# votnhan/VN_celeb_face_recognition

Hardware: AMD Instinct MI355X
Metric: embeddings/sec @ bs=256 (InceptionResnetV1, 160x160) (higher is better)
Workload: dtype bf16

## Files before the change

vn_celeb_face_recognition_amd/csrc/engine.h:

```cpp
#pragma once
#include <hip/hip_runtime.h>
#include <stdint.h>

#include <string>
#include <unordered_map>
#include <vector>

#include "../../include/vnface.h"
#include "kernels.h"

namespace vnf {

void set_error(const std::string& msg);
int fail(int code, const std::string& msg);
const char* last_error_cstr();

#define VNF_HIP(expr)                                                                         \
  do {                                                                                        \
    hipError_t _e = (expr);                                                                   \
    if (_e != hipSuccess)                                                                     \
      return ::vnf::fail(VNF_E_HIP, std::string(#expr) + ": " + hipGetErrorString(_e));       \
  } while (0)

enum class HandleKind { Encoder = 1, Mlp, Mtcnn, MlpTrainer, Retina, HeadTrainer, ConvProbe, Gallery };

struct HandleBase {
  const HandleKind kind;
  explicit HandleBase(HandleKind k) : kind(k) {}
  int device = 0;
  std::vector<void*> allocs;
  virtual ~HandleBase();
  void* dalloc(size_t bytes);
  void* upload(const void* host, size_t bytes);
};

template <class T>
T* handle_cast(vnf_handle h) {
  HandleBase* b = reinterpret_cast<HandleBase*>(h);
  return (b && b->kind == T::KIND) ? static_cast<T*>(b) : nullptr;
}

template <class T>
T* handle_cast_base(vnf_handle h) {
  HandleBase* b = reinterpret_cast<HandleBase*>(h);
  if (b)
    for (HandleKind k : T::KINDS)
      if (b->kind == k) return static_cast<T*>(b);
  return nullptr;
}

struct WeightMap {
  std::unordered_map<std::string, const vnf_tensor_desc*> m;
  std::string missing;
  WeightMap(const vnf_tensor_desc* w, int n);
  const float* get(const std::string& name, int64_t numel);
  bool has(const std::string& name) const { return m.count(name) != 0; }
};

void convert_to(int dtype, const float* src, void* dst, size_t n);

struct Buf {
  int H, W, C;
  size_t elems_per_image() const { return (size_t)H * W * C; }
  char* ptr = nullptr;
};

struct ConvLayer {
  std::string name;
  int x_buf, x_coff, cin;
  int H, W, Ho, Wo, KH, KW, sh, sw, ph, pw;
  void* w = nullptr;
  float* bias = nullptr;
  float* slope = nullptr;
  int4* ktab = nullptr;
  int K, Kpad, cout, cout_pad, ncls = 1;
  int nseg = 0;
  struct { int c0, c1, buf, coff; } seg[4];
  int res_buf = -1, res_coff = 0;
  int act = ACT_NONE, out_f32 = 0;
  int cfg = -1;
  double macs_alg = 0, macs_exec = 0;
};

struct Op {
  enum Kind { PACK, CONV, MAXPOOL, AVGPOOL, L2NORM, COPYOUT, STEM1, DWCONV, UPADD, RSTEM, DWPW, HEADS, SE } kind;
  int src = -1;
  int dst = -1, dst_coff = 0;
  int layer = -1;
  int res = -1;
  PoolWindow window = {0, 0, false};
  int frame_h = 0, frame_w = 0;
  int n_cls = 0, n_proj = 0, proj_col = 0;

  static Op pack(int dst) { Op o{PACK}; o.dst = dst; return o; }
  static Op conv(int layer) { Op o{CONV}; o.layer = layer; return o; }
  static Op stem1(int layer, int dst) { Op o{STEM1}; o.layer = layer; o.dst = dst; return o; }
  static Op maxpool(int src, int dst, int dst_coff, PoolWindow w = {3, 0, false}) {
    Op o{MAXPOOL}; o.src = src; o.dst = dst; o.dst_coff = dst_coff; o.window = w; return o;
  }
  static Op maxpool_ceil(int src, int dst, int k) { return maxpool(src, dst, 0, {k, 0, true}); }
  static Op maxpool_pad1(int src, int dst) { return maxpool(src, dst, 0, {3, 1, false}); }
  static Op avgpool(int src, int dst) { Op o{AVGPOOL}; o.src = src; o.dst = dst; return o; }
  static Op l2norm() { return Op{L2NORM}; }
  static Op copyout() { return Op{COPYOUT}; }
  static Op dwconv(int layer) { Op o{DWCONV}; o.layer = layer; return o; }
  static Op dwpw(int layer) { Op o{DWPW}; o.layer = layer; return o; }
  static Op upadd(int src, int dst) { Op o{UPADD}; o.src = src; o.dst = dst; return o; }
  static Op rstem(int frame_h, int frame_w, int dst) { Op o{RSTEM}; o.frame_h = frame_h; o.frame_w = frame_w; o.dst = dst; return o; }
  static Op se(int layer, int src, int res, int dst) { Op o{SE}; o.layer = layer; o.src = src; o.res = res; o.dst = dst; return o; }
  static Op heads(int n_cls, int n_proj, int proj_col) { Op o{HEADS}; o.n_cls = n_cls; o.n_proj = n_proj; o.proj_col = proj_col; return o; }
};

struct DwLayer {
  int x_buf, o_buf, C, stride;
  float *w = nullptr, *bias = nullptr;
  float slope = 0.f;
};

struct DwPwLayer {
  int x_buf, o_buf, cin, cout, stride;
  float *dw = nullptr, *dbias = nullptr, *pw = nullptr, *pbias = nullptr;
  float slope = 0.f;
  std::string name;
};

struct SeLayer {
  std::string name;
  int C, part_buf;
  float *w1 = nullptr, *b1 = nullptr, *w2 = nullptr, *b2 = nullptr;
  float slope_se = 0.f, slope_out = 0.f;
};

struct Group { int first, last, chunk; };

struct FusedStack {
  enum class Kind { StemMid, Block35, Block17 } kind = Kind::Block17;
  int first = 0, last = 0;
  int in_buf = -1, out_buf = -1;
  int nblocks = 0;
  int conv0 = 0;
  void* wstream = nullptr;
  float* bias = nullptr;
  void* wtail = nullptr;
  bool active = false;
  bool stack = false;
  double macs_alg = 0;
  int ext_last = 0, ext_conv = -1, ext_out_buf = -1;
  bool ext = false;
  int end() const { return ext ? ext_last : last; }
};

struct Tap { int buf, coff, C; };

struct EncoderEnv {
  int fuse = 31, direct_stem = 1, stem1a_mfma = 2, retina_fuse = 3, ws_persist = 1;
  int stem_chunk = 0, ir100_chunk1 = 0, ir100_chunk2 = 0;
  int autotune = 1, force_cfg = -2, tune_lanes = 0, autotune_log = 0;
  bool tune_final = true;
  std::string tune_cache;
  static EncoderEnv read();
};

struct RunExtra {
  float* out2 = nullptr;
  const uint8_t* prep_src = nullptr;
  int prep_s = 0;
};

constexpr int ARCH_MLP = -1, ARCH_RNET = -2, ARCH_ONET = -3, ARCH_RETINA = -5;

struct Encoder : HandleBase {
  static constexpr HandleKind KIND = HandleKind::Encoder;
  Encoder() : HandleBase(KIND) {}
  ~Encoder() override;
  int arch, dtype, max_batch, in_size;
  std::vector<Buf> bufs;
  std::vector<ConvLayer> convs;
  std::vector<DwLayer> dws;
  std::vector<DwPwLayer> dwpws;
  std::vector<SeLayer> ses;
  float *rstem_wa = nullptr, *rstem_bias = nullptr;
  std::vector<Op> ops;
  std::vector<Group> groups;
  std::vector<FusedStack> fused;
  std::vector<int> fused_at;
  int prepare_fused();
  int launch_fused(const FusedStack& f, int n0, int nn, hipStream_t s);
  std::unordered_map<std::string, Tap> taps;
  bool buf_materialised(int buf) const;
  float* emb_raw = nullptr;
  int emb_ld = 512;
  int n_cls = 0, n_proj = 0;
  float* cls_buf = nullptr;
  double macs_alg = 0, macs_exec = 0;
  Encoder* head = nullptr;
  int head_classes = 0, head_in = -1, head_logit = -1;
  float* head_emb = nullptr;
  hipEvent_t head_done = nullptr;

  int add_buf(int H, int W, int C);
  char* at(int buf, int n0, int coff = 0) const {
    return bufs[buf].ptr + ((size_t)n0 * bufs[buf].elems_per_image() + coff) * dtype_size(dtype);
  }
  float* at_f32(int buf, int n0) const { return (float*)at(buf, n0); }
  int finalize();
  int autotune();
  ConvArgs conv_args(const ConvLayer& L, int n0, int nn) const;
  int run(const void* x, int n, int x_dtype, float* out, hipStream_t s, std::string* report = nullptr,
          const RunExtra* extra = nullptr);
  int run_range(const void* x, int i0, int i1, int x_dtype, float* out, hipStream_t s, std::string* report, const RunExtra* extra);
  int write_report(std::vector<hipEvent_t>& prof_ev, const std::vector<int>& prof_op, int n, hipStream_t s, std::string* report) const;
  float* stem_wt = nullptr;
  int n_ctx = 1, next_ctx = 0;
  std::vector<std::vector<char*>> ctx_bufs;
  std::vector<float*> ctx_emb;
  std::vector<hipEvent_t> ctx_ev;
  int select_ctx(hipStream_t s, int* used);
  int max_streams = 4;
  bool tune_dirty = true;
  int tune_lanes = 1;
  int tune_batch = 0;
  const EncoderEnv env = EncoderEnv::read();
  hipStream_t side[4] = {nullptr, nullptr, nullptr, nullptr};
  hipEvent_t join_ev[4] = {nullptr, nullptr, nullptr, nullptr}, fork_ev = nullptr;
};

const char* fused_label(const FusedStack& f);
const char* fused_detail(const FusedStack& f);

int build_irv1(Encoder& e, WeightMap& wm);
int build_ir100(Encoder& e, WeightMap& wm);
int build_seir101(Encoder& e, WeightMap& wm);
int build_rn50_2b(Encoder& e, WeightMap& wm, int num_classes, int num_projections);
int build_retina_mnet(Encoder& e, WeightMap& wm, int H, int W, int head_bufs[3]);
struct NetBufs { int crops, pooled1, pooled2, heads; };
int build_rnet(Encoder& e, WeightMap& wm, bool mid, NetBufs& nb);
int build_onet(Encoder& e, WeightMap& wm, bool mid, NetBufs& nb);

}
```

vn_celeb_face_recognition_amd/csrc/fused.cpp:

```cpp
#include "engine.h"
#include "block35.h"
#include "stem_mid.h"
#include "trunk17.h"

#include <cstring>

namespace vnf {

using Kind = FusedStack::Kind;

int Encoder::prepare_fused() {
  const int enabled = env.fuse;
  for (FusedStack& f : fused) {
    f.active = false;
    if (!enabled || (dtype != BF16 && dtype != F16 && dtype != F16P) || f.nblocks < 1 || f.nblocks > T17_MAX_BLOCKS) continue;
    if (f.kind == Kind::StemMid) {
      if (!(enabled & 4)) continue;
      const ConvLayer& c2a = convs[f.conv0];
      const ConvLayer& c2b = convs[f.conv0 + 1];
      if (c2a.cout != 32 || c2a.K != 288 || c2b.cout != 64 || c2b.K != 288 || c2a.ncls != 1 || c2b.ncls != 1)
        return fail(VNF_E_INVALID, "fused stem: unexpected layer shapes");
      StemMidPack pk;
      pk.w[0] = c2a.w; pk.kpad[0] = c2a.Kpad;
      pk.w[1] = c2b.w; pk.kpad[1] = c2b.Kpad;
      bool ext_ok = false;
      if ((enabled & 8) && f.ext_conv >= 0) {
        const ConvLayer& c3b = convs[f.ext_conv];
        ext_ok = c3b.cout == 80 && c3b.K == 64 && c3b.KH == 1 && c3b.ncls == 1 && c3b.nseg == 1 && c3b.res_buf < 0 && c3b.act == ACT_RELU &&
                 bufs[f.ext_out_buf].C == 80;
      }
      if (dtype == F16P && !ext_ok) continue;
      f.wstream = dalloc(dtype == F16P ? SMS_WFRAG_BYTES : SM_WFRAG_BYTES);
      f.bias = (float*)dalloc(SM_BIAS * 4);
      if (!f.wstream || !f.bias) return VNF_E_HIP;
      VNF_HIP(hipMemcpy(f.bias, c2a.bias, 32 * 4, hipMemcpyDeviceToDevice));
      VNF_HIP(hipMemcpy(f.bias + 32, c2b.bias, 64 * 4, hipMemcpyDeviceToDevice));
      VNF_HIP(dtype == F16P ? stem_mids_repack(pk, f.wstream, 0) : stem_mid_repack(pk, f.wstream, 0));
      VNF_HIP(hipDeviceSynchronize());
      f.macs_alg = c2a.macs_alg + c2b.macs_alg;
      f.active = true;
      f.ext = ext_ok;
      if (ext_ok) f.macs_alg += convs[f.ext_conv].macs_alg;
      continue;
    }
    if (f.kind == Kind::Block35) {
      if (!(enabled & 2)) continue;
      std::vector<float> bias((size_t)f.nblocks * B35_BIAS, 0.f);
      static const int rows[5] = {96, 32, 32, 32, 256}, ks[5] = {256, 288, 288, 288, 96}, boff[5] = {0, 96, 128, 160, 192};
      const size_t wimg_bytes = dtype == F16P ? B35S_WIMG_BYTES : B35_WIMG_BYTES;
      f.wstream = dalloc((size_t)f.nblocks * wimg_bytes);
      f.bias = (float*)dalloc(bias.size() * 4);
      if (!f.wstream || !f.bias) return VNF_E_HIP;
      for (int b = 0; b < f.nblocks; ++b) {
        Block35Pack pk;
        pk.bias = f.bias + (size_t)b * B35_BIAS;
        for (int c = 0; c < 5; ++c) {
          const ConvLayer& L = convs[f.conv0 + 5 * b + c];
          if (L.cout != rows[c] || L.K != ks[c] || L.ncls != 1) return fail(VNF_E_INVALID, "fused Block35: unexpected layer shapes");
          pk.w[c] = L.w;
          pk.kpad[c] = L.Kpad;
          VNF_HIP(hipMemcpy(&bias[(size_t)b * B35_BIAS + boff[c]], L.bias, (size_t)rows[c] * 4, hipMemcpyDeviceToHost));
          f.macs_alg += L.macs_alg;
        }
        VNF_HIP(hipMemcpy(f.bias + (size_t)b * B35_BIAS, &bias[(size_t)b * B35_BIAS], (size_t)B35_BIAS * 4, hipMemcpyHostToDevice));
        VNF_HIP(dtype == F16P ? block35s_repack(pk, (char*)f.wstream + (size_t)b * wimg_bytes, 0)
                              : block35_repack(pk, (char*)f.wstream + (size_t)b * wimg_bytes, 0));
      }
      VNF_HIP(hipDeviceSynchronize());
      f.active = true;
      f.stack = (enabled & 16) && dtype != F16P;
      f.ext = false;
      if (f.stack && (enabled & 32) && f.ext_conv >= 0) {
        const ConvLayer& t = convs[f.ext_conv];
        const ConvLayer& last_up = convs[f.conv0 + 5 * (f.nblocks - 1) + 4];
        const bool ok = t.KH == 1 && t.KW == 1 && t.K == 256 && t.cout == 192 && t.ncls == 1 && t.nseg == 1 && t.res_buf < 0 &&
                        t.act == ACT_RELU && !t.out_f32 && t.x_buf == last_up.seg[0].buf && t.x_coff == 0 &&
                        t.seg[0].buf == f.ext_out_buf && t.seg[0].coff == 0 && bufs[f.ext_out_buf].C == 192;
        if (ok) {
          f.wtail = dalloc(B35_TAIL_BYTES);
          if (!f.wtail) return VNF_E_HIP;
          VNF_HIP(block35_tail_repack(t.w, t.Kpad, t.bias, f.wtail, 0));
          VNF_HIP(hipDeviceSynchronize());
          f.ext = true;
          f.macs_alg += t.macs_alg;
        }
      }
      continue;
    }
    if (!(enabled & 1)) continue;
    Trunk17Pack pk;
    memset(&pk, 0, sizeof pk);
    pk.nblocks = f.nblocks;
    std::vector<float> bias((size_t)f.nblocks * T17_BIAS, 0.f);
    static const int rows[4] = {256, 128, 128, 896}, ks[4] = {896, 896, 896, 256}, boff[4] = {0, 256, 384, 512};
    bool ok = true;
    for (int b = 0; b < f.nblocks && ok; ++b)
      for (int c = 0; c < 4 && ok; ++c) {
        const ConvLayer& L = convs[f.conv0 + 4 * b + c];
        if (L.cout != rows[c] || L.K != ks[c] || L.Kpad != ks[c] || L.ncls != 1) { ok = false; break; }
        pk.w[b][c] = L.w;
        pk.kpad[c] = L.Kpad;
        VNF_HIP(hipMemcpy(&bias[(size_t)b * T17_BIAS + boff[c]], L.bias, (size_t)rows[c] * 4, hipMemcpyDeviceToHost));
        f.macs_alg += L.macs_alg;
      }
    if (!ok) return fail(VNF_E_INVALID, "fused Block17 stack: unexpected layer shapes");
    f.wstream = dalloc(dtype == F16P ? trunk17s_stream_bytes(f.nblocks) : trunk17_stream_bytes(f.nblocks));
    f.bias = (float*)upload(bias.data(), bias.size() * 4);
    if (!f.wstream || !f.bias) return VNF_E_HIP;
    VNF_HIP(dtype == F16P ? trunk17s_repack(pk, f.wstream, 0) : trunk17_repack(pk, f.wstream, 0));
    VNF_HIP(hipDeviceSynchronize());
    f.active = true;
  }
  return VNF_OK;
}

bool Encoder::buf_materialised(int buf) const {
  for (const FusedStack& f : fused) {
    if (!f.active) continue;
    bool written = false;
    for (int oi = f.first; oi < f.end(); ++oi) {
      const Op& op = ops[oi];
      if (op.kind == Op::CONV) {
        const ConvLayer& L = convs[op.layer];
        for (int i = 0; i < L.nseg; ++i) written |= L.seg[i].buf == buf;
      } else if (op.kind == Op::MAXPOOL) {
        written |= op.dst == buf;
      }
    }
    if (!written) continue;
    bool produced = false;
    switch (f.kind) {
      case Kind::StemMid: produced = buf == (f.ext ? f.ext_out_buf : f.out_buf); break;
      case Kind::Block35:
        for (int b = 0; b < f.nblocks; ++b) produced |= convs[f.conv0 + 5 * b + 4].seg[0].buf == buf;
        produced |= f.ext && buf == f.ext_out_buf;
        break;
      case Kind::Block17: produced = buf == f.out_buf; break;
    }
    if (!produced) return false;
  }
  return true;
}

int Encoder::launch_fused(const FusedStack& f, int n0, int nn, hipStream_t s) {
  hipError_t err = hipSuccess;
  const char* what = "";
  switch (f.kind) {
    case Kind::StemMid: {
      const int out = f.ext ? f.ext_out_buf : f.out_buf;
      StemMidArgs sa;
      sa.x = at(f.in_buf, n0); sa.ldx = bufs[f.in_buf].C;
      sa.y = at(out, n0); sa.ldy = bufs[out].C;
      sa.n = nn;
      sa.wfrag = f.wstream; sa.bias = f.bias;
      sa.w3b = nullptr; sa.b3b = nullptr; sa.k3b_pad = 0;
      if (f.ext) {
        const ConvLayer& c3b = convs[f.ext_conv];
        sa.w3b = c3b.w; sa.b3b = c3b.bias; sa.k3b_pad = c3b.Kpad;
      }
      what = "fused stem";
      err = dtype == F16P ? launch_stem_mids(sa, s) : launch_stem_mid(sa, dtype, s);
      break;
    }
    case Kind::Block35:
      if (f.stack) {
        const int in = convs[f.conv0 + 4].res_buf;
        const int out = convs[f.conv0 + 5 * (f.nblocks - 1) + 4].seg[0].buf;
        Block35StackArgs ba;
        ba.x = at(in, n0); ba.ldx = bufs[in].C;
        ba.y = at(out, n0); ba.ldy = bufs[out].C;
        ba.n = nn; ba.nblocks = f.nblocks;
        ba.wimg = f.wstream;
        if (f.ext) {
          ba.wtail = f.wtail;
          ba.ytail = at(f.ext_out_buf, n0);
          ba.ldyt = bufs[f.ext_out_buf].C;
        }
        what = "fused Block35 stack";
        err = launch_block35_stack(ba, dtype, s);
        break;
      }
      what = "fused Block35";
      for (int b = 0; b < f.nblocks && err == hipSuccess; ++b) {
        const ConvLayer& up = convs[f.conv0 + 5 * b + 4];
        Block35Args ba;
        ba.x = at(up.res_buf, n0); ba.ldx = bufs[up.res_buf].C;
        ba.y = at(up.seg[0].buf, n0); ba.ldy = bufs[up.seg[0].buf].C;
        ba.n = nn;
        ba.wimg = (const char*)f.wstream + (size_t)b * (dtype == F16P ? B35S_WIMG_BYTES : B35_WIMG_BYTES);
        ba.zero = conv_zero_page();
        err = dtype == F16P ? launch_block35s(ba, s) : launch_block35(ba, dtype, s);
      }
      break;
    case Kind::Block17: {
      Trunk17Args ta;
      ta.x = at(f.in_buf, n0); ta.ldx = bufs[f.in_buf].C;
      ta.y = at(f.out_buf, n0); ta.ldy = bufs[f.out_buf].C;
      ta.n = nn; ta.nblocks = f.nblocks;
      ta.wstream = f.wstream; ta.bias = f.bias;
      what = "fused Block17 stack";
      err = dtype == F16P ? launch_trunk17s(ta, s) : launch_trunk17(ta, dtype, s);
      break;
    }
  }
  return err == hipSuccess ? VNF_OK : fail(VNF_E_HIP, std::string(what) + ": " + hipGetErrorString(err));
}

const char* fused_label(const FusedStack& f) {
  if (f.kind == Kind::StemMid) return f.ext ? "conv2d_2a+2b+maxpool_3a+3b" : "conv2d_2a+2b+maxpool_3a";
  return f.kind == Kind::Block35 ? "repeat_1 (fused blocks)" : "repeat_2 (persistent trunk)";
}

const char* fused_detail(const FusedStack& f) {
  if (f.kind == Kind::StemMid) return "rolling rows, one launch, one workgroup per image";
  if (f.kind == Kind::Block17) return "10 x Block17 in one launch, one workgroup per image";
  if (!f.stack) return "5 x Block35, one launch per block, one workgroup per image";
  return f.ext ? "5 x Block35 + mixed_6a.branch1.0 in one launch, x in registers"
               : "5 x Block35 in one launch, x in registers, one workgroup per image";
}

}
```

vn_celeb_face_recognition_amd/csrc/plan_irv1.cpp:

```cpp
#include "plan.h"

namespace vnf {

static bool basic_piece(WeightMap& wm, const std::string& p, int cin, int cout, int kh, int kw, Piece& out) {
  return fill_piece(wm, out, p + ".conv.weight", cout, cin * kh * kw, Epilogue::batchnorm(p + ".bn", 1e-3f));
}

int build_irv1(Encoder& e, WeightMap& wm) {
  e.in_size = 160;
  const int b_in = e.add_buf(160, 160, 8);
  const int b_1a = e.add_buf(79, 79, 32), b_2a = e.add_buf(77, 77, 32), b_2b = e.add_buf(77, 77, 64);
  const int b_3a = e.add_buf(38, 38, 64), b_3b = e.add_buf(38, 38, 80), b_4a = e.add_buf(36, 36, 192);
  const int x35[3] = {e.add_buf(17, 17, 256), e.add_buf(17, 17, 256), e.add_buf(17, 17, 256)};
  const int t35a = e.add_buf(17, 17, 64), t35b = e.add_buf(17, 17, 32), cat35 = e.add_buf(17, 17, 96);
  const int m6a = e.add_buf(17, 17, 192), m6b = e.add_buf(17, 17, 192);
  const int x17[3] = {e.add_buf(8, 8, 896), e.add_buf(8, 8, 896), e.add_buf(8, 8, 896)};
  const int t17a = e.add_buf(8, 8, 128), t17b = e.add_buf(8, 8, 128), cat17 = e.add_buf(8, 8, 256);
  const int m7a = e.add_buf(8, 8, 768), m7b = e.add_buf(8, 8, 256);
  const int x8[3] = {e.add_buf(3, 3, 1792), e.add_buf(3, 3, 1792), e.add_buf(3, 3, 1792)};
  const int t8a = e.add_buf(3, 3, 192), t8b = e.add_buf(3, 3, 192), cat8 = e.add_buf(3, 3, 384);
  const int pool = e.add_buf(1, 1, 1792);

  e.ops.push_back(Op::pack(b_in));

  auto simple = [&](const std::string& name, int xb, int xoff, int cin, int cin_pad, int cout, int kh, int kw, int st,
                    int ph, int pw, int ob, int ooff) -> int {
    ConvSpec s;
    s.name = name; s.x_buf = xb; s.x_coff = xoff; s.cin = cin; s.cin_pad = cin_pad;
    s.KH = kh; s.KW = kw; s.sh = s.sw = st; s.ph = ph; s.pw = pw;
    NEED(single_piece(wm, s, name + ".conv.weight", cout, ob, ooff, Epilogue::batchnorm(name + ".bn", 1e-3f)));
    return add_conv(e, s);
  };
  auto fused1x1 = [&](const std::string& name, std::vector<std::string> prefixes, int xb, int cin, int cout_each,
                      std::vector<SegSpec> segs) -> int {
    ConvSpec s;
    s.name = name; s.x_buf = xb; s.cin = s.cin_pad = cin;
    s.pieces.resize(prefixes.size());
    for (size_t i = 0; i < prefixes.size(); ++i)
      NEED(basic_piece(wm, prefixes[i], cin, cout_each, 1, 1, s.pieces[i]));
    s.segs = segs;
    return add_conv(e, s);
  };
  auto up = [&](const std::string& p, int cat, int cin, int cout, float scale, int xin, int xout, bool relu) -> int {
    ConvSpec s;
    s.name = p + ".conv2d"; s.x_buf = cat; s.cin = s.cin_pad = cin;
    NEED(single_piece(wm, s, p + ".conv2d.weight", cout, xout, 0, Epilogue::biased(p + ".conv2d.bias")));
    Piece& pc = s.pieces[0];
    pc.scale.assign(cout, scale);
    for (int i = 0; i < cout; ++i) pc.bias[i] = pc.bias[i] * scale;
    s.res_buf = xin;
    s.act = relu ? ACT_RELU : ACT_NONE;
    return add_conv(e, s);
  };

  TRY(simple("conv2d_1a", b_in, 0, 3, 8, 32, 3, 3, 2, 0, 0, b_1a, 0));
  {
    const int direct = e.env.direct_stem;
    Piece pc;
    if (direct && basic_piece(wm, "conv2d_1a", 3, 32, 3, 3, pc)) {
      std::vector<float> wt(27 * 32 + 32);
      for (int co = 0; co < 32; ++co) {
        for (int k = 0; k < 27; ++k) wt[k * 32 + co] = pc.w[co * 27 + k] * pc.scale[co];
        wt[27 * 32 + co] = pc.bias[co];
      }
      e.stem_wt = (float*)e.upload(wt.data(), wt.size() * 4);
      if (!e.stem_wt) return VNF_E_HIP;
      e.ops.resize(e.ops.size() - 2);
      e.ops.push_back(Op::stem1((int)e.convs.size() - 1, b_1a));
    }
  }
  {
    FusedStack f;
    f.kind = FusedStack::Kind::StemMid;
    f.first = (int)e.ops.size(); f.conv0 = (int)e.convs.size();
    f.in_buf = b_1a; f.out_buf = b_3a; f.nblocks = 1;
    TRY(simple("conv2d_2a", b_1a, 0, 32, 32, 32, 3, 3, 1, 0, 0, b_2a, 0));
    TRY(simple("conv2d_2b", b_2a, 0, 32, 32, 64, 3, 3, 1, 1, 1, b_2b, 0));
    e.ops.push_back(Op::maxpool(b_2b, b_3a, 0));
    f.last = (int)e.ops.size();
    TRY(simple("conv2d_3b", b_3a, 0, 64, 64, 80, 1, 1, 1, 0, 0, b_3b, 0));
    f.ext_last = (int)e.ops.size(); f.ext_conv = (int)e.convs.size() - 1; f.ext_out_buf = b_3b;
    e.fused.push_back(f);
  }
  TRY(simple("conv2d_4a", b_3b, 0, 80, 80, 192, 3, 3, 1, 0, 0, b_4a, 0));
  TRY(simple("conv2d_4b", b_4a, 0, 192, 192, 256, 3, 3, 2, 0, 0, x35[0], 0));
  const int stem_end = (int)e.ops.size();
  e.taps["conv2d_1a"] = {b_1a, 0, 32}; e.taps["conv2d_2a"] = {b_2a, 0, 32}; e.taps["conv2d_2b"] = {b_2b, 0, 64};
  e.taps["maxpool_3a"] = {b_3a, 0, 64}; e.taps["conv2d_3b"] = {b_3b, 0, 80}; e.taps["conv2d_4a"] = {b_4a, 0, 192};
  e.taps["conv2d_4b"] = {x35[0], 0, 256};

  int cur = 0;
  const int r1_first_op = (int)e.ops.size(), r1_first_conv = (int)e.convs.size();
  for (int i = 0; i < 5; ++i) {
    const std::string p = "repeat_1." + std::to_string(i);
    const int X = x35[cur], Y = x35[cur == 1 ? 2 : 1];
    TRY(fused1x1(p + ".reduce", {p + ".branch0", p + ".branch1.0", p + ".branch2.0"}, X, 256, 32,
                 {{0, 32, cat35, 0}, {32, 96, t35a, 0}}));
    TRY(simple(p + ".branch1.1", t35a, 0, 32, 32, 32, 3, 3, 1, 1, 1, cat35, 32));
    TRY(simple(p + ".branch2.1", t35a, 32, 32, 32, 32, 3, 3, 1, 1, 1, t35b, 0));
    TRY(simple(p + ".branch2.2", t35b, 0, 32, 32, 32, 3, 3, 1, 1, 1, cat35, 64));
    TRY(up(p, cat35, 96, 256, 0.17f, X, Y, true));
    cur = (cur == 1 ? 2 : 1);
  }
  e.taps["repeat_1"] = {x35[cur], 0, 256};
  {
    FusedStack f;
    f.kind = FusedStack::Kind::Block35;
    f.first = r1_first_op; f.last = (int)e.ops.size();
    f.nblocks = 5; f.conv0 = r1_first_conv;
    TRY(simple("mixed_6a.branch1.0", x35[cur], 0, 256, 256, 192, 1, 1, 1, 0, 0, m6a, 0));
    f.ext_last = (int)e.ops.size(); f.ext_conv = (int)e.convs.size() - 1; f.ext_out_buf = m6a;
    e.fused.push_back(f);
  }
  {
    const int X = x35[cur], O = x17[0];
    TRY(simple("mixed_6a.branch0", X, 0, 256, 256, 384, 3, 3, 2, 0, 0, O, 0));
    TRY(simple("mixed_6a.branch1.1", m6a, 0, 192, 192, 192, 3, 3, 1, 1, 1, m6b, 0));
    TRY(simple("mixed_6a.branch1.2", m6b, 0, 192, 192, 256, 3, 3, 2, 0, 0, O, 384));
    e.ops.push_back(Op::maxpool(X, O, 640));
  }
  e.taps["mixed_6a"] = {x17[0], 0, 896};
  cur = 0;
  const int r2_first_op = (int)e.ops.size(), r2_first_conv = (int)e.convs.size();
  for (int i = 0; i < 10; ++i) {
    const std::string p = "repeat_2." + std::to_string(i);
    const int X = x17[cur], Y = x17[cur == 1 ? 2 : 1];
    TRY(fused1x1(p + ".reduce", {p + ".branch0", p + ".branch1.0"}, X, 896, 128,
                 {{0, 128, cat17, 0}, {128, 256, t17a, 0}}));
    TRY(simple(p + ".branch1.1", t17a, 0, 128, 128, 128, 1, 7, 1, 0, 3, t17b, 0));
    TRY(simple(p + ".branch1.2", t17b, 0, 128, 128, 128, 7, 1, 1, 3, 0, cat17, 128));
    TRY(up(p, cat17, 256, 896, 0.10f, X, Y, true));
    cur = (cur == 1 ? 2 : 1);
  }
  e.taps["repeat_2"] = {x17[cur], 0, 896};
  {
    FusedStack f;
    f.kind = FusedStack::Kind::Block17;
    f.first = r2_first_op; f.last = (int)e.ops.size();
    f.in_buf = x17[0]; f.out_buf = x17[cur];
    f.nblocks = 10; f.conv0 = r2_first_conv;
    e.fused.push_back(f);
  }
  {
    const int X = x17[cur], O = x8[0];
    TRY(fused1x1("mixed_7a.reduce", {"mixed_7a.branch0.0", "mixed_7a.branch1.0", "mixed_7a.branch2.0"}, X, 896, 256,
                 {{0, 768, m7a, 0}}));
    TRY(simple("mixed_7a.branch0.1", m7a, 0, 256, 256, 384, 3, 3, 2, 0, 0, O, 0));
    TRY(simple("mixed_7a.branch1.1", m7a, 256, 256, 256, 256, 3, 3, 2, 0, 0, O, 384));
    TRY(simple("mixed_7a.branch2.1", m7a, 512, 256, 256, 256, 3, 3, 1, 1, 1, m7b, 0));
    TRY(simple("mixed_7a.branch2.2", m7b, 0, 256, 256, 256, 3, 3, 2, 0, 0, O, 640));
    e.ops.push_back(Op::maxpool(X, O, 896));
  }
  e.taps["mixed_7a"] = {x8[0], 0, 1792};
  cur = 0;
  for (int i = 0; i < 6; ++i) {
    const std::string p = i < 5 ? "repeat_3." + std::to_string(i) : std::string("block8");
    const int X = x8[cur], Y = x8[cur == 1 ? 2 : 1];
    TRY(fused1x1(p + ".reduce", {p + ".branch0", p + ".branch1.0"}, X, 1792, 192,
                 {{0, 192, cat8, 0}, {192, 384, t8a, 0}}));
    TRY(simple(p + ".branch1.1", t8a, 0, 192, 192, 192, 1, 3, 1, 0, 1, t8b, 0));
    TRY(simple(p + ".branch1.2", t8b, 0, 192, 192, 192, 3, 1, 1, 1, 0, cat8, 192));
    TRY(up(p, cat8, 384, 1792, i < 5 ? 0.20f : 1.0f, X, Y, i < 5));
    cur = (cur == 1 ? 2 : 1);
    if (i == 4) e.taps["repeat_3"] = {x8[cur], 0, 1792};
  }
  e.taps["block8"] = {x8[cur], 0, 1792};
  e.ops.push_back(Op::avgpool(x8[cur], pool));
  {
    ConvSpec s;
    s.name = "last_linear"; s.x_buf = pool; s.cin = s.cin_pad = 1792;
    NEED(single_piece(wm, s, "last_linear.weight", 512, -2, 0, Epilogue::batchnorm("last_bn", 1e-3f)));
    s.act = ACT_NONE; s.out_f32 = 1;
    TRY(add_conv(e, s));
  }
  e.ops.push_back(Op::l2norm());

  const int fuse_mask = e.env.fuse;
  int chunk = ((fuse_mask & 4) && (e.dtype == BF16 || e.dtype == F16 || (e.dtype == F16P && (fuse_mask & 8)))) ? 256 : 128;
  if (e.env.stem_chunk > 0) chunk = e.env.stem_chunk;
  e.groups.push_back({0, stem_end, chunk});
  e.groups.push_back({stem_end, (int)e.ops.size(), 1 << 30});
  return VNF_OK;
}

}
```

Before: 274,300.

## Fuse Block8 reduce, 1x3 and 3x1 convolutions into one kernel

Adds a dedicated HIP kernel that runs each Block8 branch chain (fused 1x1 reduce, 1x3 conv, 3x1 conv) in one launch. Three images share a workgroup, intermediates stay in LDS, and repacked weights stream into a register ring. A second grid row handles branch0, so the two branches run in parallel. It is enabled by default through a new fuse bit. The aim is to cut three launches per block and the global round trips of the small 3x3 intermediates, at the cost of a hand-written MFMA kernel with strict shape checks.

```diff
diff --git a/vn_celeb_face_recognition_amd/csrc/block8.h b/vn_celeb_face_recognition_amd/csrc/block8.h
--- /dev/null
+++ b/vn_celeb_face_recognition_amd/csrc/block8.h
@@ -0,0 +1,27 @@
+#pragma once
+#include <hip/hip_runtime.h>
+#include <stddef.h>
+
+namespace vnf {
+
+constexpr int B8_G = 3;
+constexpr int B8_BIAS = 768;
+
+struct Block8Args {
+  const void* x;
+  void* y;
+  int ldx, ldy, n;
+  const void* wstream;
+  const float* bias;
+};
+
+struct Block8Pack {
+  const void* w[3];
+  int kpad[3];
+};
+
+size_t block8_stream_bytes();
+hipError_t block8_repack(const Block8Pack& p, void* out, hipStream_t s);
+hipError_t launch_block8(const Block8Args& a, int dtype, hipStream_t s);
+
+}
diff --git a/vn_celeb_face_recognition_amd/csrc/block8.hip b/vn_celeb_face_recognition_amd/csrc/block8.hip
--- /dev/null
+++ b/vn_celeb_face_recognition_amd/csrc/block8.hip
@@ -0,0 +1,200 @@
+#include "block8.h"
+#include "conv_device.h"
+
+namespace vnf {
+
+namespace {
+
+constexpr int B8_ROWS = 32;
+constexpr int B8_WAVES = 12;
+constexpr int B8_RING = 8;
+constexpr int B8_KS_RED = 56;
+constexpr int B8_KS_TAP = 18;
+constexpr int B8_FRAGS0 = B8_KS_RED;
+constexpr int B8_FRAGS1 = B8_KS_RED + 2 * B8_KS_TAP;
+constexpr int B8_SLOT0 = B8_FRAGS0 + B8_RING;
+constexpr int B8_SLOT1 = B8_FRAGS1 + B8_RING;
+constexpr int B8_STREAM_FRAGS = B8_WAVES * (B8_SLOT0 + B8_SLOT1);
+constexpr int KT_BYTES = B8_ROWS * 128;
+constexpr int OFF_X = 0;
+constexpr int OFF_TA = 28 * KT_BYTES;
+constexpr int OFF_TB = 31 * KT_BYTES;
+constexpr int OFF_ZERO = 34 * KT_BYTES;
+constexpr int B8_LDS = 34 * KT_BYTES + 256;
+static_assert(B8_G * 9 <= B8_ROWS, "the group's rows fit the two pixel tiles");
+static_assert(B8_LDS <= 160 * 1024, "one workgroup's LDS");
+
+template <typename T>
+__device__ __forceinline__ uint2 bias_relu_round(const f32x4_t& acc, const f32x4_t& bias) {
+  typedef T t4 __attribute__((ext_vector_type(4)));
+  t4 o;
+#pragma unroll
+  for (int e = 0; e < 4; ++e) {
+    float v = acc[e] + bias[e];
+    v = fmaxf(v, 0.f);
+    o[e] = (T)v;
+  }
+  return __builtin_bit_cast(uint2, o);
+}
+
+}
+
+template <typename T>
+__global__ __launch_bounds__(B8_WAVES * 64) void block8_chain_kernel(const Block8Args a) {
+  extern __shared__ __attribute__((aligned(16))) char smem[];
+  const int tid = threadIdx.x, lane = tid & 63;
+  const int wave = __builtin_amdgcn_readfirstlane(tid >> 6);
+  const int frow = lane & 15, fgrp = lane >> 4;
+  const int role = 1 - (int)blockIdx.y;
+  const int img0 = blockIdx.x * B8_G;
+  const int nrows = 9 * min(B8_G, a.n - img0);
+  const unsigned lds0 = (unsigned)reinterpret_cast<uintptr_t>((__attribute__((address_space(3))) char*)smem);
+
+  const uint4* wp = reinterpret_cast<const uint4*>(a.wstream) +
+                    (size_t)(role == 0 ? wave * B8_SLOT0 : B8_WAVES * B8_SLOT0 + wave * B8_SLOT1) * 64 + lane;
+  uint4 wq[B8_RING];
+#pragma unroll
+  for (int r = 0; r < B8_RING; ++r) wq[r] = wp[r * 64];
+  wp += B8_RING * 64;
+  const int cw = 16 * wave + 4 * fgrp;
+  const f32x4_t bv_red = *reinterpret_cast<const f32x4_t*>(a.bias + role * 192 + cw);
+  f32x4_t bv_tap[2] = {bv_red, bv_red};
+  if (role == 1) {
+    bv_tap[0] = *reinterpret_cast<const f32x4_t*>(a.bias + 384 + cw);
+    bv_tap[1] = *reinterpret_cast<const f32x4_t*>(a.bias + 576 + cw);
+  }
+
+  {
+    const char* src = (const char*)a.x + (size_t)img0 * 9 * a.ldx * 2;
+    const int r = lane >> 3, slot = lane & 7;
+#pragma unroll
+    for (int i = 0; i < (112 + B8_WAVES - 1) / B8_WAVES; ++i) {
+      const int piece = wave + i * B8_WAVES;
+      if (piece < 112) {
+        const int kt = piece >> 2, rg = piece & 3;
+        const int p = min(rg * 8 + r, nrows - 1);
+        glds16(src + ((size_t)p * a.ldx + kt * 64 + ((slot ^ r) << 3)) * 2, lds0 + OFF_X + kt * KT_BYTES + rg * 1024);
+      }
+    }
+    if (tid < 16) reinterpret_cast<uint4*>(smem + OFF_ZERO)[tid] = uint4{0u, 0u, 0u, 0u};
+    asm volatile("s_waitcnt vmcnt(0)" ::: "memory");
+  }
+  __syncthreads();
+
+  const int rb0 = frow * 128 + ((fgrp ^ (frow & 7)) << 4), rb1 = rb0 ^ 64;
+  const int wb = (cw >> 6) * KT_BYTES + frow * 128 + ((((cw & 63) >> 3) ^ (frow & 7)) << 4) + (cw & 4) * 2;
+  char* yrow = (char*)a.y + ((size_t)(img0 * 9 + frow) * a.ldy + role * 192 + cw) * 2;
+
+  {
+    f32x4_t acc[2] = {f32x4_t{0.f, 0.f, 0.f, 0.f}, f32x4_t{0.f, 0.f, 0.f, 0.f}};
+#pragma unroll
+    for (int ks = 0; ks < B8_KS_RED; ++ks) {
+      uint4 xf[2];
+#pragma unroll
+      for (int i = 0; i < 2; ++i)
+        xf[i] = *reinterpret_cast<const uint4*>(smem + OFF_X + (ks >> 1) * KT_BYTES + i * 2048 + ((ks & 1) ? rb1 : rb0));
+#pragma unroll
+      for (int i = 0; i < 2; ++i) mma_chunk<T>(acc[i], wq[ks % B8_RING], xf[i]);
+      wq[ks % B8_RING] = *wp;
+      wp += 64;
+      __builtin_amdgcn_sched_barrier(0);
+    }
+    const f32x4_t bv = bv_red;
+    if (role == 0) {
+#pragma unroll
+      for (int i = 0; i < 2; ++i)
+        if (16 * i + frow < nrows) *reinterpret_cast<uint2*>(yrow + (size_t)i * 16 * a.ldy * 2) = bias_relu_round<T>(acc[i], bv);
+      return;
+    }
+#pragma unroll
+    for (int i = 0; i < 2; ++i) *reinterpret_cast<uint2*>(smem + OFF_TA + wb + i * 2048) = bias_relu_round<T>(acc[i], bv);
+  }
+  __syncthreads();
+
+  int px[2], py[2];
+#pragma unroll
+  for (int i = 0; i < 2; ++i) {
+    const int p = 16 * i + frow, q = p % 9;
+    const bool live = p < 9 * B8_G;
+    py[i] = live ? q / 3 : -8;
+    px[i] = live ? q % 3 : -8;
+  }
+#pragma unroll
+  for (int ph = 0; ph < 2; ++ph) {
+    const int src_off = ph == 0 ? OFF_TA : OFF_TB;
+    f32x4_t acc[2] = {f32x4_t{0.f, 0.f, 0.f, 0.f}, f32x4_t{0.f, 0.f, 0.f, 0.f}};
+#pragma unroll
+    for (int ks = 0; ks < B8_KS_TAP; ++ks) {
+      const int tap = ks / 6, kt = (ks % 6) >> 1, half = ks & 1;
+      uint4 xf[2];
+#pragma unroll
+      for (int i = 0; i < 2; ++i) {
+        const bool ok = (unsigned)((ph == 0 ? px[i] : py[i]) + tap - 1) < 3u;
+        const int row = 16 * i + frow + (ph == 0 ? tap - 1 : 3 * (tap - 1));
+        const int off = src_off + kt * KT_BYTES + row * 128 + (((half * 4 + fgrp) ^ (row & 7)) << 4);
+        xf[i] = *reinterpret_cast<const uint4*>(smem + (ok ? off : OFF_ZERO));
+      }
+      const int s = B8_KS_RED + B8_KS_TAP * ph + ks;
+#pragma unroll
+      for (int i = 0; i < 2; ++i) mma_chunk<T>(acc[i], wq[s % B8_RING], xf[i]);
+      wq[s % B8_RING] = *wp;
+      wp += 64;
+      __builtin_amdgcn_sched_barrier(0);
+    }
+    const f32x4_t bv = bv_tap[ph];
+    if (ph == 0) {
+#pragma unroll
+      for (int i = 0; i < 2; ++i) *reinterpret_cast<uint2*>(smem + OFF_TB + wb + i * 2048) = bias_relu_round<T>(acc[i], bv);
+      __syncthreads();
+    } else {
+#pragma unroll
+      for (int i = 0; i < 2; ++i)
+        if (16 * i + frow < nrows) *reinterpret_cast<uint2*>(yrow + (size_t)i * 16 * a.ldy * 2) = bias_relu_round<T>(acc[i], bv);
+    }
+  }
+}
+
+__global__ void block8_repack_kernel(Block8Pack p, uint4* __restrict__ out) {
+  const int lane = threadIdx.x & 63;
+  const int frag = blockIdx.x * (blockDim.x >> 6) + (threadIdx.x >> 6);
+  if (frag >= B8_STREAM_FRAGS) return;
+  int conv = -1, r0 = 0, k0 = 0;
+  if (frag < B8_WAVES * B8_SLOT0) {
+    const int wave = frag / B8_SLOT0, s = frag - wave * B8_SLOT0;
+    if (s < B8_FRAGS0) { conv = 0; r0 = 16 * wave; k0 = 32 * s; }
+  } else {
+    const int f = frag - B8_WAVES * B8_SLOT0;
+    const int wave = f / B8_SLOT1, s = f - wave * B8_SLOT1;
+    if (s < B8_KS_RED) { conv = 0; r0 = 192 + 16 * wave; k0 = 32 * s; }
+    else if (s < B8_KS_RED + B8_KS_TAP) { conv = 1; r0 = 16 * wave; k0 = 32 * (s - B8_KS_RED); }
+    else if (s < B8_FRAGS1) { conv = 2; r0 = 16 * wave; k0 = 32 * (s - B8_KS_RED - B8_KS_TAP); }
+  }
+  uint4 v = {0u, 0u, 0u, 0u};
+  if (conv >= 0)
+    v = *reinterpret_cast<const uint4*>((const char*)p.w[conv] + ((size_t)(r0 + (lane & 15)) * p.kpad[conv] + k0 + 8 * (lane >> 4)) * 2);
+  out[(size_t)frag * 64 + lane] = v;
+}
+
+size_t block8_stream_bytes() { return (size_t)B8_STREAM_FRAGS * 1024; }
+
+hipError_t block8_repack(const Block8Pack& p, void* out, hipStream_t s) {
+  hipLaunchKernelGGL(block8_repack_kernel, dim3((B8_STREAM_FRAGS + 3) / 4), dim3(256), 0, s, p, (uint4*)out);
+  return hipGetLastError();
+}
+
+hipError_t launch_block8(const Block8Args& a, int dtype, hipStream_t s) {
+  if (a.n <= 0) return hipSuccess;
+  const dim3 grid((a.n + B8_G - 1) / B8_G, 2);
+  if (dtype == BF16) {
+    allow_dynamic_lds<block8_chain_kernel<__bf16>>(B8_LDS);
+    hipLaunchKernelGGL(block8_chain_kernel<__bf16>, grid, dim3(B8_WAVES * 64), B8_LDS, s, a);
+  } else if (dtype == F16) {
+    allow_dynamic_lds<block8_chain_kernel<_Float16>>(B8_LDS);
+    hipLaunchKernelGGL(block8_chain_kernel<_Float16>, grid, dim3(B8_WAVES * 64), B8_LDS, s, a);
+  } else {
+    return hipErrorInvalidValue;
+  }
+  return hipGetLastError();
+}
+
+}
diff --git a/vn_celeb_face_recognition_amd/csrc/engine.h b/vn_celeb_face_recognition_amd/csrc/engine.h
--- a/vn_celeb_face_recognition_amd/csrc/engine.h
+++ b/vn_celeb_face_recognition_amd/csrc/engine.h
@@ -134,7 +134,8 @@
 struct Group { int first, last, chunk; };
 
 struct FusedStack {
-  enum class Kind { StemMid, Block35, Block17 } kind = Kind::Block17;
+  enum class Kind { StemMid, Block35, Block17, Block8 } kind = Kind::Block17;
+  std::string label;
   int first = 0, last = 0;
   int in_buf = -1, out_buf = -1;
   int nblocks = 0;
@@ -153,7 +154,7 @@
 struct Tap { int buf, coff, C; };
 
 struct EncoderEnv {
-  int fuse = 31, direct_stem = 1, stem1a_mfma = 2, retina_fuse = 3, ws_persist = 1;
+  int fuse = 95, direct_stem = 1, stem1a_mfma = 2, retina_fuse = 3, ws_persist = 1;
   int stem_chunk = 0, ir100_chunk1 = 0, ir100_chunk2 = 0;
   int autotune = 1, force_cfg = -2, tune_lanes = 0, autotune_log = 0;
   bool tune_final = true;
diff --git a/vn_celeb_face_recognition_amd/csrc/fused.cpp b/vn_celeb_face_recognition_amd/csrc/fused.cpp
--- a/vn_celeb_face_recognition_amd/csrc/fused.cpp
+++ b/vn_celeb_face_recognition_amd/csrc/fused.cpp
@@ -1,5 +1,6 @@
 #include "engine.h"
 #include "block35.h"
+#include "block8.h"
 #include "stem_mid.h"
 #include "trunk17.h"
 
@@ -87,6 +88,41 @@
       }
       continue;
     }
+    if (f.kind == Kind::Block8) {
+      if (!(enabled & 64) || dtype == F16P) continue;
+      const ConvLayer& red = convs[f.conv0];
+      const ConvLayer& c13 = convs[f.conv0 + 1];
+      const ConvLayer& c31 = convs[f.conv0 + 2];
+      auto plain = [](const ConvLayer& L, int cout, int K) {
+        return L.cout == cout && L.K == K && L.Kpad == K && L.ncls == 1 && L.res_buf < 0 && L.act == ACT_RELU && !L.out_f32 &&
+               L.sh == 1 && L.sw == 1 && L.H == 3 && L.W == 3 && L.Ho == 3 && L.Wo == 3;
+      };
+      const bool ok =
+          plain(red, 384, 1792) && plain(c13, 192, 576) && plain(c31, 192, 576) && f.last - f.first == 3 &&
+          red.KH == 1 && red.KW == 1 && red.x_buf == f.in_buf && red.x_coff == 0 && bufs[f.in_buf].C == 1792 && red.nseg == 2 &&
+          red.seg[0].c0 == 0 && red.seg[0].c1 == 192 && red.seg[0].buf == f.out_buf && red.seg[0].coff == 0 &&
+          red.seg[1].c0 == 192 && red.seg[1].c1 == 384 && red.seg[1].coff == 0 &&
+          c13.KH == 1 && c13.KW == 3 && c13.ph == 0 && c13.pw == 1 && c13.x_buf == red.seg[1].buf && c13.x_coff == 0 &&
+          c13.nseg == 1 && c13.seg[0].coff == 0 &&
+          c31.KH == 3 && c31.KW == 1 && c31.ph == 1 && c31.pw == 0 && c31.x_buf == c13.seg[0].buf && c31.x_coff == 0 &&
+          c31.nseg == 1 && c31.seg[0].buf == f.out_buf && c31.seg[0].coff == 192 && bufs[f.out_buf].C == 384;
+      if (!ok) return fail(VNF_E_INVALID, "fused Block8 chain: unexpected layer shapes");
+      Block8Pack pk;
+      pk.w[0] = red.w; pk.kpad[0] = red.Kpad;
+      pk.w[1] = c13.w; pk.kpad[1] = c13.Kpad;
+      pk.w[2] = c31.w; pk.kpad[2] = c31.Kpad;
+      f.wstream = dalloc(block8_stream_bytes());
+      f.bias = (float*)dalloc(B8_BIAS * 4);
+      if (!f.wstream || !f.bias) return VNF_E_HIP;
+      VNF_HIP(hipMemcpy(f.bias, red.bias, 384 * 4, hipMemcpyDeviceToDevice));
+      VNF_HIP(hipMemcpy(f.bias + 384, c13.bias, 192 * 4, hipMemcpyDeviceToDevice));
+      VNF_HIP(hipMemcpy(f.bias + 576, c31.bias, 192 * 4, hipMemcpyDeviceToDevice));
+      VNF_HIP(block8_repack(pk, f.wstream, 0));
+      VNF_HIP(hipDeviceSynchronize());
+      f.macs_alg = red.macs_alg + c13.macs_alg + c31.macs_alg;
+      f.active = true;
+      continue;
+    }
     if (!(enabled & 1)) continue;
     Trunk17Pack pk;
     memset(&pk, 0, sizeof pk);
@@ -136,6 +172,7 @@
         produced |= f.ext && buf == f.ext_out_buf;
         break;
       case Kind::Block17: produced = buf == f.out_buf; break;
+      case Kind::Block8: produced = buf == f.out_buf; break;
     }
     if (!produced) return false;
   }
@@ -202,18 +239,30 @@
       err = dtype == F16P ? launch_trunk17s(ta, s) : launch_trunk17(ta, dtype, s);
       break;
     }
+    case Kind::Block8: {
+      Block8Args ba;
+      ba.x = at(f.in_buf, n0); ba.ldx = bufs[f.in_buf].C;
+      ba.y = at(f.out_buf, n0); ba.ldy = bufs[f.out_buf].C;
+      ba.n = nn;
+      ba.wstream = f.wstream; ba.bias = f.bias;
+      what = "fused Block8 chain";
+      err = launch_block8(ba, dtype, s);
+      break;
+    }
   }
   return err == hipSuccess ? VNF_OK : fail(VNF_E_HIP, std::string(what) + ": " + hipGetErrorString(err));
 }
 
 const char* fused_label(const FusedStack& f) {
   if (f.kind == Kind::StemMid) return f.ext ? "conv2d_2a+2b+maxpool_3a+3b" : "conv2d_2a+2b+maxpool_3a";
+  if (f.kind == Kind::Block8) return f.label.c_str();
   return f.kind == Kind::Block35 ? "repeat_1 (fused blocks)" : "repeat_2 (persistent trunk)";
 }
 
 const char* fused_detail(const FusedStack& f) {
   if (f.kind == Kind::StemMid) return "rolling rows, one launch, one workgroup per image";
   if (f.kind == Kind::Block17) return "10 x Block17 in one launch, one workgroup per image";
+  if (f.kind == Kind::Block8) return "one launch, G = 3 images per workgroup, weights streamed to registers";
   if (!f.stack) return "5 x Block35, one launch per block, one workgroup per image";
   return f.ext ? "5 x Block35 + mixed_6a.branch1.0 in one launch, x in registers"
                : "5 x Block35 in one launch, x in registers, one workgroup per image";
diff --git a/vn_celeb_face_recognition_amd/csrc/plan_irv1.cpp b/vn_celeb_face_recognition_amd/csrc/plan_irv1.cpp
--- a/vn_celeb_face_recognition_amd/csrc/plan_irv1.cpp
+++ b/vn_celeb_face_recognition_amd/csrc/plan_irv1.cpp
@@ -156,10 +156,17 @@
   for (int i = 0; i < 6; ++i) {
     const std::string p = i < 5 ? "repeat_3." + std::to_string(i) : std::string("block8");
     const int X = x8[cur], Y = x8[cur == 1 ? 2 : 1];
+    FusedStack f;
+    f.kind = FusedStack::Kind::Block8;
+    f.label = p + " chain (reduce+1x3+3x1)";
+    f.first = (int)e.ops.size(); f.conv0 = (int)e.convs.size();
+    f.in_buf = X; f.out_buf = cat8; f.nblocks = 1;
     TRY(fused1x1(p + ".reduce", {p + ".branch0", p + ".branch1.0"}, X, 1792, 192,
                  {{0, 192, cat8, 0}, {192, 384, t8a, 0}}));
     TRY(simple(p + ".branch1.1", t8a, 0, 192, 192, 192, 1, 3, 1, 0, 1, t8b, 0));
     TRY(simple(p + ".branch1.2", t8b, 0, 192, 192, 192, 3, 1, 1, 1, 0, cat8, 192));
+    f.last = (int)e.ops.size();
+    e.fused.push_back(f);
     TRY(up(p, cat8, 384, 1792, i < 5 ? 0.20f : 1.0f, X, Y, i < 5));
     cur = (cur == 1 ? 2 : 1);
     if (i == 4) e.taps["repeat_3"] = {x8[cur], 0, 1792};
```

New measurement: 284,700 (median of 6 runs). +3.8%, better.
